# nightgoodl/ovmono3d

Hardware: AMD Instinct MI355X
Metric: images/sec/GPU @512x512 DINOv2-L SFP; AP3D delta vs reference (higher is better)
Workload: dtype f16x3; 1 GPU; DINOv2 vitl14 + SFP + ROIHeads3DGDINO (native GroundingDINO Swin-B/BERT-base, 900 queries, 6 categories -> NMS) + ROIAlign + CubeHead + decode, batch 1/GPU, 512x512 synthetic -> network res 532 -> canvas 896 (T=4097), random-init weights (seed 0); precision=f16x3, parallelism=dp1 (image-sharded, no data-path collective)

## Files before the change

include/ovm3d.h:

```cpp
#ifndef OVM3D_H
#define OVM3D_H

#include <stddef.h>
#include <stdint.h>

#ifdef __cplusplus
extern "C" {
#endif

#define OVM_OK 0
#define OVM_ERR_INVALID (-1)
#define OVM_ERR_HIP (-2)
#define OVM_ERR_MISSING_WEIGHT (-3)
#define OVM_ERR_SHAPE (-4)
#define OVM_ERR_CAPACITY (-5)
#define OVM_ERR_UNSUPPORTED (-6)

#define OVM_REC_FLOATS 48

typedef struct OvmHandle OvmHandle;
typedef void* ovm_stream_t;

typedef struct OvmConfig {
  int32_t embed_dim, depth, heads;
// ... 104 lines not shown
int ovm_op_gemm_swiglu(const uint16_t* a_hi, const uint16_t* a_lo, int32_t lda, const uint16_t* w_hi, const uint16_t* w_lo,
                       int32_t M, int32_t Hs, int32_t K, const float* bias, uint16_t* out_hi, uint16_t* out_lo, int32_t ldo,
                       int32_t precision, ovm_stream_t stream);
typedef struct OvmGemmEpiOp {
  int32_t epi, amode, precision, a_il, route, ksplit_hint;
  int32_t M, N, K, cH, cW, cC;
  const float* A; const float* W; const float* bias;
  const float* gamma; float* X; const int32_t* row_map; int32_t ldx, relu;
  float* C; int32_t ldc, ldo;
  float* O; int64_t o_elems; int32_t o_il, relu_o;
  const float* R; const float* R2; int32_t ldr, ldr2, padH, padW;
  float* Q; float* Kout; float* Vt; int32_t T, Tpad, heads; float qscale;
  const float* pos; int32_t G2, G, Cout, reserved;
} OvmGemmEpiOp;
int ovm_op_gemm_epi(const OvmGemmEpiOp* op, ovm_stream_t stream);
int ovm_op_interleave(const uint16_t* hi, const uint16_t* lo, int64_t rows, int32_t K, uint16_t* out, ovm_stream_t stream);
int ovm_op_layernorm(const float* x, int32_t M, int32_t D, const float* gamma, const float* beta, float eps,
                     float* y, ovm_stream_t stream);
int ovm_op_attention(const float* qkv, int32_t B, int32_t T, int32_t heads, float* out, int32_t precision,
                     ovm_stream_t stream);
int ovm_op_roi_align(const float* p2, const float* p3, const float* p4, const int32_t* hw ,
                     const float* scales , int32_t C, int32_t out_res, int32_t min_level, int32_t max_level,
                     const float* boxes, const int32_t* image_idx, int32_t n, float* out ,
                     ovm_stream_t stream);
int ovm_op_cube_decode(const float* head13, int32_t ld, const float* boxes, const float* scores, const int32_t* classes,
                       const int32_t* image_idx, const OvmImage* images, int32_t B, int32_t n, float virtual_focal,
                       int32_t postprocess, OvmDet3D* rec, int32_t* keep, ovm_stream_t stream);
int ovm_op_nms(const float* boxes, const float* scores, int32_t n, float thresh, int32_t* keep_idx, int32_t* n_keep,
               ovm_stream_t stream);
int ovm_op_rpn_proposals(const float* const* levels_o, int32_t nlev, const int32_t* sides, const float* strides,
// ... 337 lines not shown
```

ovmono3d_amd/csrc/gdino.hip:

```cpp
#include <cmath>
#include <cstdio>
#include <cstdlib>
#include "det2d.hpp"
#include "dec_chain.hpp"
#include "gdino_model.hpp"

using namespace ovm;
using namespace ovm::gdino;

namespace ovm {
GdinoTune g_gdino_tune = {1, 1, 0, 1, 1};
void set_gdino_branches(int v) { g_gdino_tune.branches = v ? 1 : 0; }
void set_gdino_dec_chain(int v) { g_gdino_tune.dec_chain = v ? 1 : 0; }
void set_gdino_ffn_split(int v) { g_gdino_tune.ffn_split = v ? 1 : 0; }
void set_gdino_swin_fused(int v) { g_gdino_tune.swin_fused = v ? 1 : 0; }
void set_gdino_gemm256(int v) { g_gdino_tune.gemm256 = v ? 1 : 0; }
}

namespace ovm {
namespace gdino {
namespace {

struct Feat { float* f; int h, w, C; };
struct DecScratch {
  float *tkv_all, *val_all;
  float *sine, *qh, *qpos, *qk, *vq, *ctx, *pre, *ow, *ffb, *b1, *b2, *delta;
  float* refs[2];
  bool chain; int ffn_chunks;
  float *ffn_x, *ffn_part;
};
struct State {
// ... 77 lines not shown
    a.scale = 1.0f / sqrtf((float)dh);
    if (r.go()) r.chk(launch_swin_qkv_attn(a, r.s_main), "swin_qkv_attn");
  } else {
    float* qkv = r.f32((size_t)M * 3 * C);
    { GemmParams q = r.gp(xw, M, blk.qkv); q.C = qkv; q.ldc = 3 * C; r.gemm(q, EPI_STORE); }
    AttnF32Params a; memset(&a, 0, sizeof(a));
    a.q = qkv; a.k = qkv + C; a.v = qkv + 2 * C; a.ldq = a.ldk = a.ldv = 3 * C;
    a.sq1 = a.sk1 = a.sv1 = (long)ws2 * 3 * C; a.sq2 = a.sk2 = a.sv2 = dh;
    a.ohi = ctx.hi; a.olo = ctx.lo; a.ldoh = ctx.ld; a.soh1 = (long)ws2 * ctx.ld; a.soh2 = dh;
    a.nb1 = nW; a.nb2 = nh; a.Tq = ws2; a.Tk = ws2; a.DH = dh; a.scale = 1.0f / sqrtf((float)dh);
    a.bias_h = blk.relbias; a.sbh = (long)ws2 * ws2; a.ldbh = ws2;
    a.bias_b = wmaps.mask; a.sbb = (long)ws2 * ws2; a.ldbb = ws2;
    r.attn(a);
  }
  { GemmParams q = r.gp(ctx, M, blk.proj); q.X = x; q.ldx = C; q.row_map = wmaps.win; r.gemm(q, EPI_RESID); }
  const bool wide = ((ntok + 127) / 128) * ((4 * C + 127) / 128) > 512 && (4 * C) % 256 == 0;
  SplitBuf hn = wide ? r.split_for256((size_t)ntok, C) : r.split((size_t)ntok, C);
  r.ln(x, ntok, C, blk.ln2, eps, nullptr, nullptr, &hn);
  SplitBuf f1 = r.split((size_t)ntok, 4 * C);
  { GemmParams q = r.gp(hn, ntok, blk.fc1); q.Ohi = f1.hi; q.Olo = f1.lo; q.ldo = f1.ld; r.gemm(q, EPI_GELU); }
  { GemmParams q = r.gp(f1, ntok, blk.fc2); q.X = x; q.ldx = C; r.gemm(q, EPI_RESID); }
  r.release(mk);
}

float* patch_merge(Run& r, const SwinStage& stg, const StageGeo& ge, const float* x, int C) {
  const int h2 = ge.h2, w2 = ge.w2;
  float* xn = r.f32((size_t)h2 * w2 * 2 * C);
  const size_t mk = r.mark();
  SplitBuf xm = r.split((size_t)h2 * w2, 4 * C);
  RowOpParams p = Run::rows(x, C, h2 * w2, 4 * C); Run::into(p, xm);
// ... 54 lines not shown
    RowOpParams p = Run::rows(f.f, f.C, n, K); Run::into(p, a);
    if (conv) { p.idx = pl->conv_map; p.nidx = 9; p.seg = f.C; }
    r.rowop(p);
    GemmParams q = r.gp(a, n, g->inproj[l].w); q.C = y; q.ldc = D;
    r.gemm(q, EPI_STORE);
    if (r.go()) r.chk(ovm_g_groupnorm(y, 1, n, D, 32, g->inproj[l].gn.g, g->inproj[l].gn.b, 1e-5f, st.vis0 + (size_t)pl->lstart[l] * D, r.s_main), "groupnorm");
  }
  r.release(mk);
}

struct EncBufs {
  float* v; SplitBuf vsp; float *t, *qvv, *tkv; SplitBuf cv; float* ct;
  BiAttnWs bw; float *sc, *stat, *part, *bml;
  float *text2, *tqk, *tv, *tctx, *tff;
  SplitBuf vis_sp, visp_sp; float *val, *ow; SplitBuf dsp; float* pre; SplitBuf ff;
};

void fusion_layer(Run& r, const EncLayer& ly, EncBufs& b, const float* vis_in, const float* text_in) {
  const OvmGdinoConfig& c = r.g->cfg;
  const int D = c.d_model, T = r.pl->T, S = r.pl->S, HF = c.heads / 2, E = c.ffn_dim / 2, dhf = E / HF;
  r.ln(vis_in, S, D, ly.lnv, c.eps, nullptr, b.v, &b.vsp);
  r.ln(text_in, T, D, ly.lnt, c.eps, nullptr, b.t);
  { GemmParams q = r.gp(b.vsp, S, ly.vqv); q.C = b.qvv; q.ldc = 2 * E; r.gemm(q, EPI_STORE); }
  r.lin(b.t, nullptr, D, T, ly.tkv, 0, nullptr, 0, b.tkv, 2 * E);
  if (!r.go()) return;
  BiAttnParams a; memset(&a, 0, sizeof(a));
  a.qv = b.qvv; a.ldq = 2 * E; a.kt = b.tkv; a.ldk = 2 * E; a.vv = b.qvv + E; a.ldvv = 2 * E; a.vt = b.tkv + E; a.ldvt = 2 * E;
  a.S = S; a.T = T; a.H = HF; a.dh = dhf; a.scale = 1.0f / sqrtf((float)dhf);
  a.cv_hi = b.cv.hi; a.cv_lo = b.cv.lo; a.ldcv = b.cv.ld; a.ct = b.ct; a.sc = b.sc; a.stat = b.stat; a.part = b.part; a.chunk = b.bw.chunk; a.nchunk = b.bw.nchunk;
  if (b.bml) { a.bm = b.bml; a.bl = b.bml + b.bw.ml; }
// ... 18 lines not shown

void deformable_layer(Run& r, const EncLayer& ly, EncBufs& b, float* vis) {
  const OvmGdinoConfig& c = r.g->cfg; Plan* pl = r.pl;
  const int D = c.d_model, S = pl->S, NOW = now_cols(c);
  { GemmParams q = r.gp(b.cv, S, ly.ov); q.C = vis; q.ldc = D; q.R = b.v; q.ldr = D; r.gemm(q, EPI_STORE); }
  {
    RowOpParams p = Run::rows(vis, D, S, D); Run::into(p, b.vis_sp);
    p.add = pl->pos; p.ld_add = D; p.add_rows = S; p.hi2 = b.visp_sp.hi; p.lo2 = b.visp_sp.lo; p.ldh2 = b.visp_sp.ld;
    r.rowop(p);
  }
  { GemmParams q = r.gp(b.vis_sp, S, ly.msda.value); q.C = b.val; q.ldc = D; r.gemm(q, EPI_STORE); }
  { GemmParams q = r.gp(b.visp_sp, S, ly.msda.offw); q.C = b.ow; q.ldc = NOW; r.gemm(q, EPI_STORE); }
  deform(r, b.val, D, b.ow, NOW, pl->ref, 2, 0, S, nullptr, &b.dsp);
  { GemmParams q = r.gp(b.dsp, S, ly.msda.out); q.C = b.pre; q.ldc = D; q.R = vis; q.ldr = D; r.gemm(q, EPI_STORE); }
  r.ln(b.pre, S, D, ly.de_ln1, c.eps, nullptr, b.v, &b.vsp);
  { GemmParams q = r.gp(b.vsp, S, ly.de_fc1); q.Ohi = b.ff.hi; q.Olo = b.ff.lo; q.ldo = b.ff.ld; q.relu = 1; r.gemm(q, EPI_STORE); }
  { GemmParams q = r.gp(b.ff, S, ly.de_fc2); q.C = b.pre; q.ldc = D; q.R = b.v; q.ldr = D; r.gemm(q, EPI_STORE); }
  r.ln(b.pre, S, D, ly.de_ln2, c.eps, nullptr, vis);
}

void encoder(Run& r, State& st) {
  const OvmGdinoConfig& c = r.g->cfg;
  const int D = c.d_model, T = r.pl->T, S = r.pl->S, HF = c.heads / 2, E = c.ffn_dim / 2, dhf = E / HF;
  r.join();
  const size_t mk = r.mark();
  EncBufs b;
  b.v = r.f32((size_t)S * D); b.vsp = r.split_for256((size_t)S, D);
  b.t = r.f32((size_t)T * D);
  b.qvv = r.f32((size_t)S * 2 * E);
  b.tkv = r.f32((size_t)T * 2 * E);
  b.cv = r.split((size_t)S, E);
  b.ct = r.f32((size_t)T * E);
  b.bw = biattn_workspace(S, T, HF, dhf, false);
  b.sc = b.bw.sc ? r.f32(b.bw.sc) : nullptr;
  b.stat = b.bw.stat ? r.f32(b.bw.stat) : nullptr;
  b.part = r.f32(b.bw.part);
  b.bml = b.bw.ml ? r.f32(2 * b.bw.ml) : nullptr;
  b.text2 = r.f32((size_t)T * D);
  b.tqk = r.f32((size_t)T * 2 * D); b.tv = r.f32((size_t)T * D); b.tctx = r.f32((size_t)T * D);
  b.tff = r.f32((size_t)T * c.ffn_dim);
  b.vis_sp = r.split((size_t)S, D); b.visp_sp = r.split((size_t)S, D);
  b.val = r.f32((size_t)S * D);
  b.ow = r.f32((size_t)S * now_cols(c));
  b.dsp = r.split((size_t)S, D);
  b.pre = r.f32((size_t)S * D);
  b.ff = r.split((size_t)S, c.ffn_dim);
  const float* vis_in = st.vis0; const float* text_in = st.text0;
  for (auto& ly : r.g->enc) {
    fusion_layer(r, ly, b, vis_in, text_in);
    vis_in = st.vis; text_in = st.text;
    text_enhancer(r, ly, b, st.text);
    deformable_layer(r, ly, b, st.vis);
    r.join();
  }
  r.release(mk);
  r.tap("source_flatten", st.vis0, (int64_t)S * D);
  r.tap("enc_vision", st.vis, (int64_t)S * D);
  r.tap("enc_text", st.text, (int64_t)T * D);
}

void select_queries(Run& r, State& st) {
// ... 292 lines not shown
    if (r) { delete pl; return r; }
    pl->arena_cap = dry.peak + 4096;
    void* q = nullptr;
    if (hipMalloc(&q, pl->arena_cap) != hipSuccess) { delete pl; g->err = "arena allocation failed"; return OVM_ERR_HIP; }
    pl->allocs.push_back(q); pl->arena = (char*)q; pl->bytes += pl->arena_cap;
    evict_plans(g, pl);
  }
  g->plans.push_front(pl);
  g->last = pl;
  OVM_TRY(g, ovm_g_normalize_image(image, g->cfg.pixel_mean, g->cfg.pixel_std, g->cfg.flip_channels, pl->img, s));
  if (pl->exec) {
    OVM_HIP(g, hipGraphLaunch(pl->exec, s));
  } else {
    Run run{g, pl, s, false};
    OVM_TRY(g, forward_impl(run));
    pl->launches = run.launches;
    if (g->graphs_enabled) capture_plan(g, pl, s);
  }
  g->launches_last = pl->launches;
  const size_t nl = (size_t)g->cfg.num_queries * g->cfg.max_text_len;
  if (pred_logits) OVM_HIP(g, hipMemcpyAsync(pred_logits, pl->out_logits, nl * sizeof(float), hipMemcpyDeviceToDevice, s));
  if (pred_boxes) OVM_HIP(g, hipMemcpyAsync(pred_boxes, pl->out_boxes, (size_t)g->cfg.num_queries * 4 * sizeof(float), hipMemcpyDeviceToDevice, s));
  return OVM_OK;
}

int ovm_gdino_detect(OvmGdino* g, const OvmImage* image, const int32_t* token_ids, int32_t ntok, const int32_t* spans, int32_t n_phrases,
                     float box_threshold, float nms_threshold, float* out_boxes, float* out_scores, int32_t* out_classes, int32_t* n_out,
                     ovm_stream_t stream) {
  int r = ovm_gdino_forward(g, image, token_ids, ntok, nullptr, nullptr, nullptr, stream);
  if (r) return r;
  Plan* pl = g->last;
// ... 2 lines not shown
}

int32_t ovm_gdino_num_queries(const OvmGdino* g) { return g ? g->cfg.num_queries : 0; }

int ovm_gdino_last_outputs(OvmGdino* g, const float** pred_logits, const float** pred_boxes, int32_t* logits_ld) {
  if (!g || !g->last) return OVM_ERR_INVALID;
  if (pred_logits) *pred_logits = g->last->out_logits;
  if (pred_boxes) *pred_boxes = g->last->out_boxes;
  if (logits_ld) *logits_ld = g->cfg.max_text_len;
  return OVM_OK;
}

int64_t ovm_gdino_debug_copy(OvmGdino* g, const char* name, void* dst, int64_t capacity_elems, ovm_stream_t stream) {
  if (!g || !g->last || !name) return OVM_ERR_INVALID;
  if (std::string(name) == "launches") return g->launches_last;
  if (std::string(name) == "plans") return (int64_t)g->plans.size();
  if (std::string(name) == "plan_bytes") { int64_t b = 0; for (Plan* q : g->plans) b += (int64_t)q->bytes; return b; }
  auto it = g->last->taps.find(name);
  if (it == g->last->taps.end()) { g->err = std::string("unknown debug tensor ") + name; return OVM_ERR_INVALID; }
  if (it->second.second > capacity_elems) return OVM_ERR_CAPACITY;
  if (hipMemcpyAsync(dst, it->second.first, (size_t)it->second.second * 4, hipMemcpyDeviceToDevice, (hipStream_t)stream) != hipSuccess) return OVM_ERR_HIP;
  return it->second.second;
}

}
```

ovmono3d_amd/csrc/gdino.hpp:

```cpp
#pragma once
#include "common.hpp"
#include "kernels.hpp"

namespace ovm {

struct RowOpParams {
  const float* x; int ldx;
  const int* idx; int nidx; int seg;
  const float* res; int ldr;
  const float* gamma; const float* beta; float eps;
  int zero_masked;
  const float* add; int ld_add; int add_rows;
  int M, D;
  float* y; int ldy;
  float* y2; int ldy2;
  half_t* hi; half_t* lo; int ldh;
  int il;
  half_t* hi2; half_t* lo2; int ldh2;
};
int launch_rowop(const RowOpParams& p, hipStream_t s);

struct AttnF32Params {
  const float *q, *k, *v; int ldq, ldk, ldv;
  long sq1, sq2, sk1, sk2, sv1, sv2;
// ... 8 lines not shown
int launch_attn_f32(const AttnF32Params& p, hipStream_t s);

struct SwinQkvAttnParams {
  const half_t* xhi; const half_t* xlo; int ldx;
  const half_t* wfrag; int KS;
  const float* bias;
  int C, nh, nW;
  const float* relbias;
  const float* mask;
  half_t* ohi; half_t* olo; int ldo;
  float scale;
};
bool swin_qkv_attn_supported(int C, int nh, int ws, int npass);
int launch_swin_qkv_attn(const SwinQkvAttnParams& p, hipStream_t s);

int launch_relpos_tables(const float* q, int ldq, int M, int H, int DH, int gh, int gw, const float* Rh, const float* Rw, float* rel_h,
                         float* rel_w, int ldrel, hipStream_t s);

struct BiAttnParams {
  const float* qv; int ldq;
  const float* kt; int ldk;
  const float* vv; int ldvv;
  const float* vt; int ldvt;
  int S, T, H, dh; float scale;
  half_t* cv_hi; half_t* cv_lo; int ldcv;
  float* cv;
  float* ct;
  float* sc;
  float* stat;
  float* part;
// ... 31 lines not shown
```

ovmono3d_amd/csrc/gdino_model.hpp:

```cpp
#pragma once
#include <hip/hip_runtime.h>
#include <array>
#include <cstring>
#include <list>
#include <map>
#include <string>
#include <vector>
#include "../../include/ovm3d.h"
#include "gdino.hpp"
#include "kernels.hpp"
#include "loader.hpp"
#include "tower.hpp"

namespace ovm {

struct GdinoTune {
  int branches;
  int dec_chain;
  int ffn_split;
  int swin_fused;
  int gemm256;
};
extern GdinoTune g_gdino_tune;

namespace gdino {

struct Lin : PackedLin {
  half_t* frag = nullptr;
  std::vector<half_t> img;
};
struct Ln { float* g = nullptr; float* b = nullptr; };
struct SplitBuf { half_t* hi = nullptr; half_t* lo = nullptr; int ld = 0; bool il = false; };

struct SwinBlock { Ln ln1, ln2; Lin qkv, proj, fc1, fc2; float* relbias = nullptr; };
struct SwinStage { std::vector<SwinBlock> blocks; int nh = 0, C = 0; bool has_red = false; Lin red; Ln dn; bool has_out = false; Ln on; };
struct BertLayer { Lin qkv, ao, fi, fo; Ln aln, oln; };
// ... 59 lines not shown
  std::vector<void*> allocs; size_t bytes = 0;
  int* d_ids = nullptr; int* d_pids = nullptr; float* text_bias = nullptr; float* text_pos = nullptr;
  int Hp = 0, Wp = 0; int* pe_map = nullptr;
  std::vector<StageGeo> geo;
  int nlev = 0; int lh[8] = {0}, lw[8] = {0}, lstart[8] = {0}; int S = 0;
  int* conv_map = nullptr; int conv_h = 0, conv_w = 0;
  float* pos = nullptr; float* ref = nullptr; float* prop_logit = nullptr; int* valid_idx = nullptr;
  float* img = nullptr;
  char* arena = nullptr; size_t arena_cap = 0;
  float* gemm_ws = nullptr; size_t gemm_ws_cap = 0;
  unsigned long long* topk_keys = nullptr; int topk_N = 0;
  float* out_logits = nullptr; float* out_boxes = nullptr;
  std::map<std::string, std::pair<const void*, int64_t>> taps;
  hipGraph_t graph = nullptr; hipGraphExec_t exec = nullptr;
  long launches = 0;
  void drop_graph() {
    if (exec) { (void)hipGraphExecDestroy(exec); exec = nullptr; }
    if (graph) { (void)hipGraphDestroy(graph); graph = nullptr; }
  }
  ~Plan() {
    drop_graph();
    for (void* p : allocs) (void)hipFree(p);
  }
};

int build_plan(OvmGdino* g, int H, int W, const std::vector<int>& ids, const std::vector<int>& pids, Plan** out);
Plan* find_plan(OvmGdino* g, int H, int W, const std::vector<int>& ids, const std::vector<int>& pids);
void evict_plans(OvmGdino* g, const Plan* incoming);
void capture_plan(OvmGdino* g, Plan* pl, hipStream_t s);

constexpr size_t kAuxWs = (size_t)16 << 20;

struct Run {
  OvmGdino* g; Plan* pl; hipStream_t s; bool dry;
  size_t off = 0, peak = 0;
  long launches = 0;
  int rc = OVM_OK;
  hipStream_t s_main = nullptr;
  float* ws = nullptr; size_t ws_cap = 0;
  bool two() const { return g->branches && g->aux && !dry; }
  void init_streams() { s_main = s; ws = pl->gemm_ws; ws_cap = two() ? pl->gemm_ws_cap - kAuxWs : pl->gemm_ws_cap; }
  void fork() {
    if (!two() || rc != OVM_OK) return;
    if (hipEventRecord(g->ev_fork, s_main) != hipSuccess || hipStreamWaitEvent(g->aux, g->ev_fork, 0) != hipSuccess) fail(OVM_ERR_HIP, "fork");
  }
  void on_text() { if (two()) { s = g->aux; ws = (float*)((char*)pl->gemm_ws + (pl->gemm_ws_cap - kAuxWs)); ws_cap = kAuxWs; } }
  void on_image() { if (two()) { s = s_main; ws = pl->gemm_ws; ws_cap = pl->gemm_ws_cap - kAuxWs; } }
  void join() {
    if (!two()) return;
    on_image();
    if (rc != OVM_OK) return;
// ... 15 lines not shown
    const size_t bytes = rows * b.ld * sizeof(half_t);
    b.hi = (half_t*)alloc(bytes);
    b.lo = g->precision == 3 ? (half_t*)alloc(bytes) : nullptr;
    if (b.ld != K && go()) {
      if (hipMemsetAsync(b.hi, 0, bytes, s) != hipSuccess) fail(OVM_ERR_HIP, "memset");
      if (b.lo && hipMemsetAsync(b.lo, 0, bytes, s) != hipSuccess) fail(OVM_ERR_HIP, "memset");
    }
    return b;
  }
  SplitBuf split_for256(size_t rows, int K) {
    if (g->precision != 3 || K % 32 || !pl->tune.gemm256) return split(rows, K);
    SplitBuf b; b.il = true; b.ld = 2 * K;
    b.hi = (half_t*)alloc(rows * b.ld * sizeof(half_t)); b.lo = b.hi ? b.hi + 32 : nullptr;
    return b;
  }
  size_t mark() const { return off; }
  void release(size_t m) { off = m; }
  void fail(int r, const char* what) { if (rc == OVM_OK) { rc = r; if (g->err.empty()) g->err = what; } }
  void chk(int r, const char* what) { ++launches; if (r != OVM_OK) fail(r, what); }
  void tap(const std::string& name, const void* p, int64_t n) { if (!dry) pl->taps[name] = {p, n}; }

  bool go() const { return !dry && rc == OVM_OK; }
  void copy(void* dst, const void* src, size_t bytes, hipStream_t st) {
    if (go() && hipMemcpyAsync(dst, src, bytes, hipMemcpyDeviceToDevice, st) != hipSuccess) fail(OVM_ERR_HIP, "hipMemcpyAsync");
  }
  static RowOpParams rows(const float* x, int ldx, int M, int D) {
    RowOpParams p; memset(&p, 0, sizeof(p));
    p.x = x; p.ldx = ldx; p.M = M; p.D = D;
    return p;
  }
  static void into(RowOpParams& p, const SplitBuf& b) { p.hi = b.hi; p.lo = b.lo; p.ldh = b.ld; p.il = b.il ? 1 : 0; }
  void rowop(const RowOpParams& p) { if (go()) chk(launch_rowop(p, s), "rowop"); }

  GemmParams gp(const SplitBuf& A, int M, const Lin& W) {
    GemmParams p = gp_base(SplitImg{A.hi, A.lo}, A.ld, W, M);
    p.a_il = A.il ? 1 : 0; p.ws_slot = 1; p.part_ws = ws; p.part_cap = ws_cap;
    return p;
  }
  void gemm(const GemmParams& p, int epi) {
    if (!go()) return;
    if (p.a_il && gemm256_supported(p, g->precision)) chk(launch_gemm256(p, epi, 1, s), "gemm256");
    else chk(launch_gemm(p, g->precision, epi, A_ROWMAJOR, s), "gemm");
  }

  void lin(const float* A, const float* A2, int lda, int M, const Lin& W, int act, const float* R, int ldr, float* C, int ldc) {
    if (!go() || M <= 0) return;
    if (!gemm_small_supported(A, lda, W.K) || (A2 && (((uintptr_t)A2) & 15))) { fail(OVM_ERR_SHAPE, "lin: unaligned fp32 operand"); return; }
    chk(launch_gemm_small_ex(A, A2, lda, M, W.K, W.hi, W.lo, W.N, W.Kpad, W.bias, act, R, ldr, C, ldc, g->precision, ws, ws_cap, s),
        "lin");
  }
  void ln(const float* x, int M, int D, const Ln& w, float eps, const float* res, float* y, const SplitBuf* sp = nullptr) {
    RowOpParams p = rows(x, D, M, D);
    p.res = res; p.ldr = D; p.gamma = w.g; p.beta = w.b; p.eps = eps; p.y = y; p.ldy = D;
    if (sp) into(p, *sp);
    rowop(p);
  }
  void attn(const AttnF32Params& p) { if (go()) chk(launch_attn_f32(p, s), "attn_f32"); }
};

// ... 5 lines not shown
```

ovmono3d_amd/csrc/ops.hip:

```cpp
#include <hip/hip_runtime.h>
#include <cstring>
#include <vector>
#include "../../include/ovm3d.h"
#include "kernels.hpp"
#include "det2d.hpp"
#include "tower.hpp"

using namespace ovm;

namespace {
__global__ void split_kernel(const float* __restrict__ x, int64_t n, half_t* __restrict__ hi, half_t* __restrict__ lo) {
  const int64_t i = (int64_t)blockIdx.x * blockDim.x + threadIdx.x;
  if (i >= n) return;
  half_t h, l; split_f16(x[i], h, l);
  hi[i] = h;
  if (lo) lo[i] = l;
}
__global__ void qkv_layout_kernel(const float* __restrict__ qkv, int B, int T, int Tpad, int heads,
                                  half_t* Qh, half_t* Ql, half_t* Kh, half_t* Kl, half_t* Vh, half_t* Vl) {
  const int D = heads * 64;
  const int64_t i = (int64_t)blockIdx.x * blockDim.x + threadIdx.x;
  const int64_t total = (int64_t)B * T * 3 * D;
  if (i >= total) return;
  const int n = (int)(i % (3 * D)); const int64_t m = i / (3 * D);
// ... 16 lines not shown
  y[i] = (float)hi[i] + (lo ? (float)lo[i] : 0.f);
}
struct Tmp {
  std::vector<void*> p;
  template <typename Tp> Tp* get(size_t n, bool zero = false) {
    void* q = nullptr;
    if (hipMalloc(&q, n * sizeof(Tp) + 16) != hipSuccess) return nullptr;
    if (zero) hipMemset(q, 0, n * sizeof(Tp) + 16);
    p.push_back(q);
    return (Tp*)q;
  }
  ~Tmp() { for (void* q : p) hipFree(q); }
};
}

namespace ovm { void set_use_gemm256(int v); void set_gdino_branches(int v); void msdeform_set_vec(int v); void set_gdino_dec_chain(int v); void set_gdino_gemm256(int v); void set_gdino_swin_fused(int v); void set_gdino_ffn_split(int v); void gemm256_set_n192(int v); void set_gemm256_ksplit(int v); }

extern "C" {

int ovm_op_split_f16(const float* x, int64_t n, uint16_t* hi, uint16_t* lo, ovm_stream_t stream) {
  if (n <= 0) return OVM_OK;
  hipLaunchKernelGGL(split_kernel, dim3((unsigned)((n + 255) / 256)), dim3(256), 0, (hipStream_t)stream, x, n, (half_t*)hi, (half_t*)lo);
  return hipGetLastError() == hipSuccess ? OVM_OK : OVM_ERR_HIP;
}

static int g_op_gemm256 = 0;
static unsigned long long* g_gemm256_stamps = nullptr;

int ovm_op_gemm(const uint16_t* a_hi, const uint16_t* a_lo, int32_t lda, const uint16_t* w_hi, const uint16_t* w_lo,
                int32_t M, int32_t N, int32_t K, const float* bias, int32_t relu, float* c, int32_t ldc,
                int32_t precision, ovm_stream_t stream) {
// ... 131 lines not shown
  if (d->epi == EPI_QKV) {
    const int64_t bh = (int64_t)((d->M + d->T - 1) / d->T) * d->heads, nqk = bh * d->T * 64, nv = bh * 64 * d->Tpad;
    if (nv < 1) return OVM_ERR_INVALID;
    Out* q = add_out(d->Q, nqk, split); Out* k = add_out(d->Kout, nqk, split); Out* v = add_out(d->Vt, nv, split);
    if (!q || !k || !v) return OVM_ERR_HIP;
    p.Qhi = q->hi; p.Qlo = q->lo; p.Khi = k->hi; p.Klo = k->lo; p.Vhi = v->hi; p.Vlo = v->lo;
  }
  const int rc = d->route == 1 ? launch_gemm256(p, d->epi, d->ksplit_hint, s) : launch_gemm(p, d->precision, d->epi, d->amode, s);
  if (rc == OVM_OK)
    for (int i = 0; i < n_out; ++i)
      hipLaunchKernelGGL(join_kernel, grid1d(outs[i].n), dim3(256), 0, s, outs[i].hi, outs[i].lo, outs[i].n, outs[i].f);
  if (hipStreamSynchronize(s) != hipSuccess) return OVM_ERR_HIP;
  return rc;
}

int ovm_op_interleave(const uint16_t* hi, const uint16_t* lo, int64_t rows, int32_t K, uint16_t* out, ovm_stream_t stream) {
  if (rows <= 0) return OVM_OK;
  if (!hi || !lo || !out || K % 32 != 0) return OVM_ERR_INVALID;
  const long n = (long)rows * K;
  hipLaunchKernelGGL(interleave_kernel, dim3((unsigned)((n + 255) / 256)), dim3(256), 0, (hipStream_t)stream, (const half_t*)hi, (const half_t*)lo,
                     (long)rows, K, (half_t*)out);
  return hipGetLastError() == hipSuccess ? OVM_OK : OVM_ERR_HIP;
}

int ovm_op_layernorm(const float* x, int32_t M, int32_t D, const float* gamma, const float* beta, float eps, float* y,
                     ovm_stream_t stream) {
  LnOut o; memset(&o, 0, sizeof(o)); o.f32 = y; o.ldf = D;
  return launch_ln_rows(x, D, M, D, gamma, beta, eps, o, (hipStream_t)stream);
}

// ... 137 lines not shown
}

int ovm_tune_set(const char* key, int32_t value) {
  if (!key) return OVM_ERR_INVALID;
  if (!strcmp(key, "gemm_bm")) { gemm_set_force_bm(value); return OVM_OK; }
  if (!strcmp(key, "gemm_stages")) { gemm_set_stages(value); return OVM_OK; }
  if (!strcmp(key, "gemm_splitk")) { gemm_set_splitk(value); return OVM_OK; }
  if (!strcmp(key, "gemm_tail")) { gemm_set_tail_rows(value); return OVM_OK; }
  if (!strcmp(key, "attn_waves")) { attn_set_waves(value); return OVM_OK; }
  if (!strcmp(key, "attn_pp")) {
#ifndef OVM_DIAG
    if (value < 0 || value > 1) return OVM_ERR_INVALID;
#endif
    attn_set_pp(value); return OVM_OK;
  }
  if (!strcmp(key, "gdino_ffn_split")) { ovm::set_gdino_ffn_split(value); return OVM_OK; }
  if (!strcmp(key, "gdino_swin_fused")) { ovm::set_gdino_swin_fused(value); return OVM_OK; }
  if (!strcmp(key, "gdino_gemm256")) { ovm::set_gdino_gemm256(value); return OVM_OK; }
  if (!strcmp(key, "gdino_dec_chain")) { ovm::set_gdino_dec_chain(value); return OVM_OK; }
  if (!strcmp(key, "msdeform_vec")) { msdeform_set_vec(value); return OVM_OK; }
  if (!strcmp(key, "attn_q64")) { attn_set_q64(value); return OVM_OK; }
  if (!strcmp(key, "attn_prio")) { attn_set_prio(value); return OVM_OK; }
  if (!strcmp(key, "attn_lds_pad")) { attn_set_lds_pad(value); return OVM_OK; }
  if (!strcmp(key, "attn_tail")) { attn_set_tail_rows(value); return OVM_OK; }
  if (!strcmp(key, "attn_tail_split")) { attn_set_tail_split(value); return OVM_OK; }
  if (!strcmp(key, "glin_small_max_tiles")) { glinear_set_small_max_tiles(value); return OVM_OK; }
  if (!strcmp(key, "glin_target_blocks")) { gemm_small_set(value, -1); return OVM_OK; }
  if (!strcmp(key, "gbmm_tiled")) { gbmm_set_tiled(value); return OVM_OK; }
  if (!strcmp(key, "glin_stages")) { gemm_small_set_stages(value); return OVM_OK; }
  if (!strcmp(key, "glin_wpe")) { gemm_small_set_wpe(value); return OVM_OK; }
// ... 91 lines not shown
```

ovmono3d_amd/lib.py:

```python
from __future__ import annotations

import ctypes as C
import os
from typing import Dict, Iterable, List, Optional, Sequence

import numpy as np

_HERE = os.path.dirname(os.path.abspath(__file__))
LIB_PATH = os.path.join(_HERE, "libovm3d.so")

OVM_REC_FLOATS = 48


class OvmConfig(C.Structure):
    _fields_ = [
        ("embed_dim", C.c_int32), ("depth", C.c_int32), ("heads", C.c_int32),
        ("pos_grid", C.c_int32), ("canvas", C.c_int32), ("fpn_channels", C.c_int32),
        ("use_depth_fusion", C.c_int32),
        ("pixel_mean", C.c_float * 3), ("pixel_std", C.c_float * 3),
        ("num_classes", C.c_int32), ("fc_dim", C.c_int32), ("pooler_res", C.c_int32),
        ("pooler_min_level", C.c_int32), ("pooler_max_level", C.c_int32),
        ("virtual_focal", C.c_float),
        ("anchor_sizes", C.c_float * 4), ("anchor_ratios", C.c_float * 3),
        ("rpn_pre_topk", C.c_int32), ("rpn_post_topk", C.c_int32), ("rpn_nms_thresh", C.c_float),
# ... 174 lines not shown
class OvmRowOp(C.Structure):
    _fields_ = [
        ("x", C.c_void_p), ("idx", C.c_void_p), ("res", C.c_void_p), ("gamma", C.c_void_p), ("beta", C.c_void_p), ("add", C.c_void_p),
        ("ldx", C.c_int32), ("nidx", C.c_int32), ("seg", C.c_int32), ("ldr", C.c_int32), ("eps", C.c_float),
        ("zero_masked", C.c_int32), ("ld_add", C.c_int32), ("add_rows", C.c_int32),
        ("M", C.c_int32), ("D", C.c_int32),
        ("y", C.c_void_p), ("y2", C.c_void_p), ("hi", C.c_void_p), ("lo", C.c_void_p), ("hi2", C.c_void_p), ("lo2", C.c_void_p),
        ("ldy", C.c_int32), ("ldy2", C.c_int32), ("ldh", C.c_int32), ("il", C.c_int32), ("ldh2", C.c_int32), ("reserved0", C.c_int32),
    ]


EXPORTS = [
    "ovm_create", "ovm_destroy", "ovm_last_error", "ovm_version", "ovm_abi_sizeof", "ovm_backbone_forward", "ovm_cube_forward",
    "ovm_rpn_box_forward", "ovm_gather_records", "ovm_gather_counts", "ovm_host_interp_pos_embed", "ovm_host_resize_pos_embed_aa", "ovm_host_sincos_pos_embed", "ovm_host_shard_range",
    "ovm_backbone_num_levels", "ovm_backbone_level",
    "ovm_op_split_f16", "ovm_op_interleave", "ovm_op_gemm", "ovm_op_gemm_epi", "ovm_op_gemm_swiglu", "ovm_host_swiglu_perm", "ovm_op_layernorm", "ovm_op_attention", "ovm_op_roi_align",
    "ovm_op_roi_align_ex", "ovm_op_compact_records", "ovm_op_ln_rows", "ovm_op_ln_gelu_split", "ovm_op_patch_gather", "ovm_op_patch_gather_f32",
    "ovm_op_cls_init", "ovm_op_tokens_cast", "ovm_op_tokens_writeback", "ovm_op_maxpool2",
    "ovm_op_cube_decode", "ovm_op_nms", "ovm_op_rpn_proposals", "ovm_op_boxhead_post", "ovm_debug_copy", "ovm_set_corun", "ovm_profile_enable", "ovm_profile_read",
    "ovm_comm_unique_id", "ovm_comm_init", "ovm_comm_destroy", "ovm_tune_set", "ovm_gdino_postprocess", "ovm_box3d_iou", "ovm_eval_iou2d", "ovm_eval_match", "ovm_eval_iou3d", "ovm_eval_nhd", "ovm_host_pil_bilinear_coeffs", "ovm_resize_bilinear_u8", "ovm_resize_bilinear_f32",
    "ovm_g_pack_weight", "ovm_host_pack_weight", "ovm_g_linear", "ovm_g_layernorm", "ovm_g_bmm", "ovm_g_bmm2", "ovm_g_softmax", "ovm_g_softmax2", "ovm_g_eltwise", "ovm_g_gather_rows",
    "ovm_g_groupnorm", "ovm_g_biattn", "ovm_g_msdeform", "ovm_g_sine_embed", "ovm_g_normalize_image", "ovm_g_topk", "ovm_g_rowmax",
    "ovm_g_attn_f32", "ovm_g_msdeform_fused", "ovm_g_rowop",
    "ovm_gdino_create", "ovm_gdino_destroy", "ovm_gdino_last_error", "ovm_gdino_forward", "ovm_gdino_detect", "ovm_gdino_set_force_topk",
    "ovm_gdino_debug_copy", "ovm_debug_set_ptr", "ovm_gdino_num_queries", "ovm_gdino_last_outputs", "ovm_infer",
    "ovm_host_jpeg_info", "ovm_host_jpeg_entropy_decode", "ovm_jpeg_reconstruct",
    "ovm_host_scene_layout", "ovm_render_scene_workspace", "ovm_render_scene",
    "ovm_geo_default_params", "ovm_geo_last_error", "ovm_geo_lift_workspace", "ovm_geo_lift", "ovm_geo_dbscan_workspace", "ovm_geo_dbscan",
    "ovm_host_geo_box",
    "ovm_sam_create", "ovm_sam_destroy", "ovm_sam_last_error", "ovm_sam_set_image", "ovm_sam_predict_boxes_workspace", "ovm_sam_predict_boxes",
    "ovm_sam_debug_copy",
# ... 39 lines not shown
    lib.ovm_backbone_forward.argtypes = [vp, C.POINTER(OvmImage), i32, vp, i32, i32, vp, vp, vp, vp]
    lib.ovm_cube_forward.argtypes = [vp, C.POINTER(OvmImage), i32, vp, vp, vp, vp, i32, i32, vp, vp, vp]
    lib.ovm_rpn_box_forward.argtypes = [vp, C.POINTER(OvmImage), i32, vp, vp, vp, vp, vp, vp, vp]
    lib.ovm_gather_records.argtypes = [vp, i32, i32, vp, i32, vp, C.POINTER(i32), vp]
    lib.ovm_gather_counts.argtypes = [vp, i32, i32, i32, C.POINTER(i32), vp]
    lib.ovm_host_interp_pos_embed.argtypes = [vp, i32, i32, i32, vp]
    lib.ovm_host_resize_pos_embed_aa.argtypes = [vp, i32, i32, i32, vp]
    lib.ovm_host_sincos_pos_embed.argtypes = [i32, i32, vp]
    lib.ovm_backbone_num_levels.argtypes = [vp]
    lib.ovm_backbone_level.argtypes = [vp, i32, C.POINTER(vp), C.POINTER(i32), C.POINTER(f32)]
    lib.ovm_host_shard_range.argtypes = [i64, i32, i32, C.POINTER(i64), C.POINTER(i64)]
    lib.ovm_op_split_f16.argtypes = [vp, i64, vp, vp, vp]
    lib.ovm_op_interleave.argtypes = [vp, vp, i64, i32, vp, vp]
    lib.ovm_op_gemm.argtypes = [vp, vp, i32, vp, vp, i32, i32, i32, vp, i32, vp, i32, i32, vp]
    lib.ovm_op_gemm_epi.argtypes = [C.POINTER(OvmGemmEpiOp), vp]
    lib.ovm_op_gemm_swiglu.argtypes = [vp, vp, i32, vp, vp, i32, i32, i32, vp, vp, vp, i32, i32, vp]
    lib.ovm_host_swiglu_perm.argtypes = [i32, vp]
    lib.ovm_op_layernorm.argtypes = [vp, i32, i32, vp, vp, f32, vp, vp]
    lib.ovm_op_attention.argtypes = [vp, i32, i32, i32, vp, i32, vp]
    lib.ovm_op_roi_align.argtypes = [vp, vp, vp, C.POINTER(i32), C.POINTER(f32), i32, i32, i32, i32, vp, vp, i32, vp, vp]
    lib.ovm_op_cube_decode.argtypes = [vp, i32, vp, vp, vp, vp, C.POINTER(OvmImage), i32, i32, f32, i32, vp, vp, vp]
    lib.ovm_op_roi_align_ex.argtypes = [C.POINTER(vp), i32, C.POINTER(i32), C.POINTER(f32), i32, i32, i32, i32, vp, vp, i32, vp, vp, i32, vp]
    lib.ovm_op_compact_records.argtypes = [vp, vp, i32, i32, vp, vp, vp]
    lib.ovm_op_ln_rows.argtypes = [vp, i32, i32, i32, vp, vp, f32, vp, i32, vp, vp, i32, i32, i32, i32, vp]
    lib.ovm_op_ln_gelu_split.argtypes = [vp, vp, i32, i32, vp, vp, f32, vp]
    lib.ovm_op_patch_gather.argtypes = [C.POINTER(OvmImage), i32, i32, i32, i32, C.POINTER(f32), C.POINTER(f32), vp, vp, vp]
    lib.ovm_op_patch_gather_f32.argtypes = [C.POINTER(i64), i32, i32, i32, vp, vp, vp]
    lib.ovm_op_cls_init.argtypes = [vp, vp, vp, vp, i32, i32, i32, i32, vp]
    lib.ovm_op_tokens_cast.argtypes = [vp, i32, i32, i32, i32, i32, vp, vp, vp, vp]
    lib.ovm_op_tokens_writeback.argtypes = [vp, vp, i32, i32, i32, i32, vp]
# ... 140 lines not shown
```

Baseline: 51.56 images/sec.

## Fuse GroundingDINO FFN fc1+activation+fc2 into one split-hidden MFMA kernel

Adds a fused MLP kernel that computes fc1, bias and GELU/ReLU, and the fc2 partial product per 256-wide hidden chunk. The hidden activation stays in LDS, and chunk partials are reduced by the existing split-K epilogue. It is used for small Swin block MLPs and for the encoder deformable FFN when the shape limits (at most 96 output tiles) and the workspace allow, removing the round trip of the wide hidden tensor through global memory and one GEMM launch. In exchange it writes fp32 partials of size chunks×M×C, reloads the input tile once per hidden chunk, and relies on a hand-written double-buffered pipeline.

```diff
diff --git a/include/ovm3d.h b/include/ovm3d.h
--- a/include/ovm3d.h
+++ b/include/ovm3d.h
@@ -142,6 +142,9 @@
   const float* pos; int32_t G2, G, Cout, reserved;
 } OvmGemmEpiOp;
 int ovm_op_gemm_epi(const OvmGemmEpiOp* op, ovm_stream_t stream);
+int ovm_op_mlp_fused(const uint16_t* x_il, int32_t ldx, const uint16_t* w1_il, const float* b1, const uint16_t* w2_il, const float* b2,
+                     int32_t M, int32_t C, int32_t hidden, int32_t act, float* ws, int64_t ws_bytes, float* X, const float* R, float* Y,
+                     ovm_stream_t stream);
 int ovm_op_interleave(const uint16_t* hi, const uint16_t* lo, int64_t rows, int32_t K, uint16_t* out, ovm_stream_t stream);
 int ovm_op_layernorm(const float* x, int32_t M, int32_t D, const float* gamma, const float* beta, float eps,
                      float* y, ovm_stream_t stream);
diff --git a/ovmono3d_amd/csrc/gdino.hip b/ovmono3d_amd/csrc/gdino.hip
--- a/ovmono3d_amd/csrc/gdino.hip
+++ b/ovmono3d_amd/csrc/gdino.hip
@@ -9,12 +9,13 @@
 using namespace ovm::gdino;
 
 namespace ovm {
-GdinoTune g_gdino_tune = {1, 1, 0, 1, 1};
+GdinoTune g_gdino_tune = {1, 1, 0, 1, 1, 1};
 void set_gdino_branches(int v) { g_gdino_tune.branches = v ? 1 : 0; }
 void set_gdino_dec_chain(int v) { g_gdino_tune.dec_chain = v ? 1 : 0; }
 void set_gdino_ffn_split(int v) { g_gdino_tune.ffn_split = v ? 1 : 0; }
 void set_gdino_swin_fused(int v) { g_gdino_tune.swin_fused = v ? 1 : 0; }
 void set_gdino_gemm256(int v) { g_gdino_tune.gemm256 = v ? 1 : 0; }
+void set_gdino_mlp_fused(int v) { g_gdino_tune.mlp_fused = v < 0 ? 0 : (v > 2 ? 2 : v); }
 }
 
 namespace ovm {
@@ -122,6 +123,14 @@
     r.attn(a);
   }
   { GemmParams q = r.gp(ctx, M, blk.proj); q.X = x; q.ldx = C; q.row_map = wmaps.win; r.gemm(q, EPI_RESID); }
+  if (r.mlp_fused_ok(1, ntok, blk.fc1, blk.fc2, 2)) {
+    SplitBuf hn = r.split_il((size_t)ntok, C);
+    r.ln(x, ntok, C, blk.ln2, eps, nullptr, nullptr, &hn);
+    GemmParams q = r.gp(hn, ntok, blk.fc2); q.X = x; q.ldx = C;
+    r.mlp_fused(hn, ntok, blk.fc1, blk.fc2, 2, q, EPI_RESID);
+    r.release(mk);
+    return;
+  }
   const bool wide = ((ntok + 127) / 128) * ((4 * C + 127) / 128) > 512 && (4 * C) % 256 == 0;
   SplitBuf hn = wide ? r.split_for256((size_t)ntok, C) : r.split((size_t)ntok, C);
   r.ln(x, ntok, C, blk.ln2, eps, nullptr, nullptr, &hn);
@@ -206,6 +215,7 @@
   BiAttnWs bw; float *sc, *stat, *part, *bml;
   float *text2, *tqk, *tv, *tctx, *tff;
   SplitBuf vis_sp, visp_sp; float *val, *ow; SplitBuf dsp; float* pre; SplitBuf ff;
+  bool ffn_fused;
 };
 
 void fusion_layer(Run& r, const EncLayer& ly, EncBufs& b, const float* vis_in, const float* text_in) {
@@ -254,8 +264,13 @@
   deform(r, b.val, D, b.ow, NOW, pl->ref, 2, 0, S, nullptr, &b.dsp);
   { GemmParams q = r.gp(b.dsp, S, ly.msda.out); q.C = b.pre; q.ldc = D; q.R = vis; q.ldr = D; r.gemm(q, EPI_STORE); }
   r.ln(b.pre, S, D, ly.de_ln1, c.eps, nullptr, b.v, &b.vsp);
-  { GemmParams q = r.gp(b.vsp, S, ly.de_fc1); q.Ohi = b.ff.hi; q.Olo = b.ff.lo; q.ldo = b.ff.ld; q.relu = 1; r.gemm(q, EPI_STORE); }
-  { GemmParams q = r.gp(b.ff, S, ly.de_fc2); q.C = b.pre; q.ldc = D; q.R = b.v; q.ldr = D; r.gemm(q, EPI_STORE); }
+  if (b.ffn_fused) {
+    GemmParams q = r.gp(b.vsp, S, ly.de_fc2); q.C = b.pre; q.ldc = D; q.R = b.v; q.ldr = D;
+    r.mlp_fused(b.vsp, S, ly.de_fc1, ly.de_fc2, 1, q, EPI_STORE);
+  } else {
+    { GemmParams q = r.gp(b.vsp, S, ly.de_fc1); q.Ohi = b.ff.hi; q.Olo = b.ff.lo; q.ldo = b.ff.ld; q.relu = 1; r.gemm(q, EPI_STORE); }
+    { GemmParams q = r.gp(b.ff, S, ly.de_fc2); q.C = b.pre; q.ldc = D; q.R = b.v; q.ldr = D; r.gemm(q, EPI_STORE); }
+  }
   r.ln(b.pre, S, D, ly.de_ln2, c.eps, nullptr, vis);
 }
 
@@ -284,7 +299,9 @@
   b.ow = r.f32((size_t)S * now_cols(c));
   b.dsp = r.split((size_t)S, D);
   b.pre = r.f32((size_t)S * D);
-  b.ff = r.split((size_t)S, c.ffn_dim);
+  b.ffn_fused = b.vsp.il;
+  for (auto& ly : r.g->enc) b.ffn_fused = b.ffn_fused && r.mlp_fused_ok(2, S, ly.de_fc1, ly.de_fc2, 1);
+  if (!b.ffn_fused) b.ff = r.split((size_t)S, c.ffn_dim);
   const float* vis_in = st.vis0; const float* text_in = st.text0;
   for (auto& ly : r.g->enc) {
     fusion_layer(r, ly, b, vis_in, text_in);
@@ -607,7 +624,7 @@
   } else {
     Run run{g, pl, s, false};
     OVM_TRY(g, forward_impl(run));
-    pl->launches = run.launches;
+    pl->launches = run.launches; pl->mlp_fused_sites = run.mlp_sites;
     if (g->graphs_enabled) capture_plan(g, pl, s);
   }
   g->launches_last = pl->launches;
@@ -640,6 +657,7 @@
 int64_t ovm_gdino_debug_copy(OvmGdino* g, const char* name, void* dst, int64_t capacity_elems, ovm_stream_t stream) {
   if (!g || !g->last || !name) return OVM_ERR_INVALID;
   if (std::string(name) == "launches") return g->launches_last;
+  if (std::string(name) == "mlp_fused_sites") return g->last->mlp_fused_sites;
   if (std::string(name) == "plans") return (int64_t)g->plans.size();
   if (std::string(name) == "plan_bytes") { int64_t b = 0; for (Plan* q : g->plans) b += (int64_t)q->bytes; return b; }
   auto it = g->last->taps.find(name);
diff --git a/ovmono3d_amd/csrc/gdino.hpp b/ovmono3d_amd/csrc/gdino.hpp
--- a/ovmono3d_amd/csrc/gdino.hpp
+++ b/ovmono3d_amd/csrc/gdino.hpp
@@ -46,6 +46,18 @@
 bool swin_qkv_attn_supported(int C, int nh, int ws, int npass);
 int launch_swin_qkv_attn(const SwinQkvAttnParams& p, hipStream_t s);
 
+struct MlpFusedParams {
+  const half_t* X; int ldx;
+  const half_t* W1; const float* b1;
+  const half_t* W2;
+  int M, C, hidden;
+  int act;
+  float* part; size_t part_cap;
+};
+bool mlp_fused_supported(int M, int C, int hidden, int act, int npass);
+size_t mlp_fused_ws_bytes(int M, int C, int hidden);
+int launch_mlp_fused(const MlpFusedParams& p, const GemmParams& out, int epi, hipStream_t s);
+
 int launch_relpos_tables(const float* q, int ldq, int M, int H, int DH, int gh, int gw, const float* Rh, const float* Rw, float* rel_h,
                          float* rel_w, int ldrel, hipStream_t s);
 
diff --git a/ovmono3d_amd/csrc/gdino_model.hpp b/ovmono3d_amd/csrc/gdino_model.hpp
--- a/ovmono3d_amd/csrc/gdino_model.hpp
+++ b/ovmono3d_amd/csrc/gdino_model.hpp
@@ -20,6 +20,7 @@
   int ffn_split;
   int swin_fused;
   int gemm256;
+  int mlp_fused;
 };
 extern GdinoTune g_gdino_tune;
 
@@ -109,6 +110,7 @@
   std::map<std::string, std::pair<const void*, int64_t>> taps;
   hipGraph_t graph = nullptr; hipGraphExec_t exec = nullptr;
   long launches = 0;
+  int mlp_fused_sites = 0;
   void drop_graph() {
     if (exec) { (void)hipGraphExecDestroy(exec); exec = nullptr; }
     if (graph) { (void)hipGraphDestroy(graph); graph = nullptr; }
@@ -130,6 +132,7 @@
   OvmGdino* g; Plan* pl; hipStream_t s; bool dry;
   size_t off = 0, peak = 0;
   long launches = 0;
+  int mlp_sites = 0;
   int rc = OVM_OK;
   hipStream_t s_main = nullptr;
   float* ws = nullptr; size_t ws_cap = 0;
@@ -175,6 +178,11 @@
     b.hi = (half_t*)alloc(rows * b.ld * sizeof(half_t)); b.lo = b.hi ? b.hi + 32 : nullptr;
     return b;
   }
+  SplitBuf split_il(size_t rows, int K) {
+    SplitBuf b; b.il = true; b.ld = 2 * K;
+    b.hi = (half_t*)alloc(rows * b.ld * sizeof(half_t)); b.lo = b.hi + 32;
+    return b;
+  }
   size_t mark() const { return off; }
   void release(size_t m) { off = m; }
   void fail(int r, const char* what) { if (rc == OVM_OK) { rc = r; if (g->err.empty()) g->err = what; } }
@@ -204,6 +212,23 @@
     else chk(launch_gemm(p, g->precision, epi, A_ROWMAJOR, s), "gemm");
   }
 
+  bool mlp_fused_ok(int site, int M, const Lin& fc1, const Lin& fc2, int act) const {
+    const int C = fc2.N, hidden = fc1.N;
+    if (pl->tune.mlp_fused < site || g->precision != 3 || fc1.K != C || fc1.Kpad != C || fc2.K != hidden || fc2.Kpad != hidden) return false;
+    if (!mlp_fused_supported(M, C, hidden, act, g->precision)) return false;
+    if ((long)((M + 127) / 128) * ((C + 127) / 128) > 96) return false;
+    const size_t cap = (g->branches && g->aux) ? pl->gemm_ws_cap - kAuxWs : pl->gemm_ws_cap;
+    return mlp_fused_ws_bytes(M, C, hidden) <= cap;
+  }
+  void mlp_fused(const SplitBuf& A, int M, const Lin& fc1, const Lin& fc2, int act, const GemmParams& out, int epi) {
+    ++mlp_sites;
+    if (!go()) return;
+    MlpFusedParams p; memset(&p, 0, sizeof(p));
+    p.X = A.hi; p.ldx = A.ld; p.W1 = fc1.hi; p.b1 = fc1.bias; p.W2 = fc2.hi; p.M = M; p.C = fc2.N; p.hidden = fc1.N; p.act = act;
+    p.part = ws; p.part_cap = ws_cap;
+    chk(launch_mlp_fused(p, out, epi, s), "mlp_fused");
+  }
+
   void lin(const float* A, const float* A2, int lda, int M, const Lin& W, int act, const float* R, int ldr, float* C, int ldc) {
     if (!go() || M <= 0) return;
     if (!gemm_small_supported(A, lda, W.K) || (A2 && (((uintptr_t)A2) & 15))) { fail(OVM_ERR_SHAPE, "lin: unaligned fp32 operand"); return; }
diff --git a/ovmono3d_amd/csrc/mlp_fused.hip b/ovmono3d_amd/csrc/mlp_fused.hip
--- /dev/null
+++ b/ovmono3d_amd/csrc/mlp_fused.hip
@@ -0,0 +1,189 @@
+#include <hip/hip_runtime.h>
+#include "gemm.hpp"
+#include "gdino.hpp"
+
+namespace ovm {
+
+namespace {
+
+constexpr int kBM = 64;
+constexpr int kHC = 256;
+constexpr int kKG = kHC / 32;
+constexpr int kBN = 256;
+constexpr int kSlot = (kBM + 256) * 128;
+constexpr int kOffW = kBM * 128;
+constexpr int kOffH = 2 * kSlot;
+constexpr int kHGroup = kBM * 128;
+constexpr int kSmem = kOffH + kKG * kHGroup;
+static_assert(kSmem <= 160 * 1024 && kSlot % 16 == 0 && kOffH % 16 == 0, "LDS map");
+
+__device__ __forceinline__ int frag_off(int row, int chunk) { return row * 128 + (chunk ^ ((row >> 1) & 7)) * 16; }
+
+template <int ACT>
+__global__ __launch_bounds__(512) void mlp_fused_kernel(const MlpFusedParams p) {
+  extern __shared__ __attribute__((aligned(16))) char smem[];
+  const int tid = threadIdx.x, lane = tid & 63;
+  const int wave = __builtin_amdgcn_readfirstlane(tid >> 6);
+  const int chunks = p.hidden / kHC;
+  const int chunk = (int)blockIdx.x % chunks, m0 = ((int)blockIdx.x / chunks) * kBM;
+  const int N = p.C;
+  const int S1 = p.C / 32;
+  const int S = S1 + ((N + kBN - 1) / kBN) * kKG;
+  const size_t ldw1 = 2 * (size_t)p.C, ldw2 = 2 * (size_t)p.hidden;
+
+  const int srow = lane >> 3, sslot = lane & 7;
+  size_t aoff, w1off[4];
+  int w2row[4], w2col[4];
+  {
+    const int row = wave * 8 + srow;
+    int m = m0 + row; if (m > p.M - 1) m = p.M - 1;
+    aoff = (size_t)m * p.ldx + (sslot ^ ((row >> 1) & 7)) * 8;
+  }
+#pragma unroll
+  for (int q = 0; q < 4; ++q) {
+    const int row = (wave + 8 * q) * 8 + srow;
+    const int ch = sslot ^ ((row >> 1) & 7);
+    w1off[q] = (size_t)(chunk * kHC + row) * ldw1 + ch * 8;
+    w2row[q] = row;
+    w2col[q] = chunk * kKG * 64 + ch * 8;
+  }
+  auto stage = [&](int s) {
+    char* base = smem + (s & 1) * kSlot;
+    if (s < S1) {
+      glds16(p.X + aoff + (size_t)s * 64, base + wave * 1024);
+#pragma unroll
+      for (int q = 0; q < 4; ++q) glds16(p.W1 + w1off[q] + (size_t)s * 64, base + kOffW + (wave + 8 * q) * 1024);
+    } else {
+      const int s2 = s - S1, nb = s2 / kKG, g = s2 % kKG;
+#pragma unroll
+      for (int q = 0; q < 4; ++q) {
+        int n = nb * kBN + w2row[q]; if (n > N - 1) n = N - 1;
+        glds16(p.W2 + (size_t)n * ldw2 + w2col[q] + g * 64, base + kOffW + (wave + 8 * q) * 1024);
+      }
+    }
+  };
+
+  const int fr = lane & 15, fq = lane >> 4;
+  const int wm = wave >> 2, wn = wave & 3;
+  int oa_hi[2], oa_lo[2], ow_hi[4], ow_lo[4];
+#pragma unroll
+  for (int mi = 0; mi < 2; ++mi) {
+    const int row = wm * 32 + mi * 16 + fr;
+    oa_hi[mi] = frag_off(row, fq); oa_lo[mi] = frag_off(row, 4 + fq);
+  }
+#pragma unroll
+  for (int ni = 0; ni < 4; ++ni) {
+    const int row = wn * 64 + ni * 16 + fr;
+    ow_hi[ni] = kOffW + frag_off(row, fq); ow_lo[ni] = kOffW + frag_off(row, 4 + fq);
+  }
+  f32x4 acc[2][4];
+  auto zero = [&]() {
+#pragma unroll
+    for (int mi = 0; mi < 2; ++mi)
+#pragma unroll
+      for (int ni = 0; ni < 4; ++ni) acc[mi][ni] = (f32x4){0.f, 0.f, 0.f, 0.f};
+  };
+  auto mma = [&](const char* abase, const char* wbase) {
+    half8 ah[2], al[2], wh[4], wl[4];
+#pragma unroll
+    for (int mi = 0; mi < 2; ++mi) { ah[mi] = *(const half8*)(abase + oa_hi[mi]); al[mi] = *(const half8*)(abase + oa_lo[mi]); }
+#pragma unroll
+    for (int ni = 0; ni < 4; ++ni) { wh[ni] = *(const half8*)(wbase + ow_hi[ni]); wl[ni] = *(const half8*)(wbase + ow_lo[ni]); }
+#pragma unroll
+    for (int ni = 0; ni < 4; ++ni)
+#pragma unroll
+      for (int mi = 0; mi < 2; ++mi) {
+        f32x4 c = acc[mi][ni];
+        c = __builtin_amdgcn_mfma_f32_16x16x32_f16(wl[ni], ah[mi], c, 0, 0, 0);
+        c = __builtin_amdgcn_mfma_f32_16x16x32_f16(wh[ni], al[mi], c, 0, 0, 0);
+        c = __builtin_amdgcn_mfma_f32_16x16x32_f16(wh[ni], ah[mi], c, 0, 0, 0);
+        acc[mi][ni] = c;
+      }
+  };
+
+  zero();
+  stage(0);
+  asm volatile("s_waitcnt vmcnt(0)" ::: "memory");
+  __syncthreads();
+  for (int s = 0; s < S; ++s) {
+    if (s + 1 < S) stage(s + 1);
+    const char* slot = smem + (s & 1) * kSlot;
+    if (s < S1) {
+      mma(slot, slot);
+      if (s == S1 - 1) {
+#pragma unroll
+        for (int ni = 0; ni < 4; ++ni) {
+          const int hc = wn * 64 + ni * 16 + fq * 4;
+          const f32x4 b = p.b1 ? *(const f32x4*)(p.b1 + chunk * kHC + hc) : (f32x4){0.f, 0.f, 0.f, 0.f};
+          char* hg = smem + kOffH + (hc >> 5) * kHGroup + (fq & 1) * 8;
+          const int c = (ni & 1) * 2 + (fq >> 1);
+#pragma unroll
+          for (int mi = 0; mi < 2; ++mi) {
+            const int row = wm * 32 + mi * 16 + fr;
+            half4 h, l;
+#pragma unroll
+            for (int r = 0; r < 4; ++r) {
+              const float z = acc[mi][ni][r] + b[r];
+              half_t hh, ll; split_f16(ACT == 2 ? gelu_erf(z) : fmaxf(z, 0.f), hh, ll); h[r] = hh; l[r] = ll;
+            }
+            *(half4*)(hg + frag_off(row, c)) = h;
+            *(half4*)(hg + frag_off(row, 4 + c)) = l;
+          }
+        }
+        zero();
+      }
+    } else {
+      const int s2 = s - S1, nb = s2 / kKG, g = s2 % kKG;
+      mma(smem + kOffH + g * kHGroup, slot);
+      if (g == kKG - 1) {
+#pragma unroll
+        for (int mi = 0; mi < 2; ++mi) {
+          const int m = m0 + wm * 32 + mi * 16 + fr;
+#pragma unroll
+          for (int ni = 0; ni < 4; ++ni) {
+            const int n = nb * kBN + wn * 64 + ni * 16 + fq * 4;
+            if (m < p.M && n < N) *(f32x4*)(p.part + ((size_t)chunk * p.M + m) * N + n) = acc[mi][ni];
+          }
+        }
+        zero();
+      }
+    }
+    asm volatile("s_waitcnt vmcnt(0)" ::: "memory");
+    __syncthreads();
+  }
+}
+
+}
+
+bool mlp_fused_supported(int M, int C, int hidden, int act, int npass) {
+  return npass == 3 && M >= 1 && C >= 32 && C % 32 == 0 && hidden >= kHC && hidden % kHC == 0 && (act == 1 || act == 2) &&
+         ((long)(M + kBM - 1) / kBM) * (hidden / kHC) <= 0x7fffffffL;
+}
+
+size_t mlp_fused_ws_bytes(int M, int C, int hidden) { return (size_t)(hidden / kHC) * M * C * sizeof(float); }
+
+int launch_mlp_fused(const MlpFusedParams& p, const GemmParams& out, int epi, hipStream_t s) {
+  if (!mlp_fused_supported(p.M, p.C, p.hidden, p.act, 3) || (epi != EPI_RESID && epi != EPI_STORE)) return OVM_ERR_INVALID;
+  if (!p.X || !p.W1 || !p.W2 || !p.part || p.ldx < 2 * p.C || p.ldx % 8 != 0) return OVM_ERR_INVALID;
+  if ((((uintptr_t)p.X) | ((uintptr_t)p.W1) | ((uintptr_t)p.W2) | ((uintptr_t)p.part) | ((uintptr_t)p.b1)) & 15) return OVM_ERR_INVALID;
+  if (epi == EPI_RESID ? !out.X : (!out.C && !out.Ohi)) return OVM_ERR_INVALID;
+  if (p.part_cap < mlp_fused_ws_bytes(p.M, p.C, p.hidden)) return OVM_ERR_CAPACITY;
+  const int chunks = p.hidden / kHC, tiles = (p.M + kBM - 1) / kBM;
+  static bool attr_set = false;
+  if (!attr_set) {
+    if (hipFuncSetAttribute((const void*)mlp_fused_kernel<1>, hipFuncAttributeMaxDynamicSharedMemorySize, kSmem) != hipSuccess ||
+        hipFuncSetAttribute((const void*)mlp_fused_kernel<2>, hipFuncAttributeMaxDynamicSharedMemorySize, kSmem) != hipSuccess)
+      return OVM_ERR_HIP;
+    attr_set = true;
+  }
+  if (p.act == 2) hipLaunchKernelGGL((mlp_fused_kernel<2>), dim3(tiles * chunks), dim3(512), kSmem, s, p);
+  else hipLaunchKernelGGL((mlp_fused_kernel<1>), dim3(tiles * chunks), dim3(512), kSmem, s, p);
+  GemmParams q = out;
+  q.M = p.M; q.N = p.C; q.K = p.hidden; q.ksplit = chunks; q.kchunk = kKG; q.part = p.part;
+  const long n = (long)p.M * (p.C / 4);
+  if (epi == EPI_RESID) hipLaunchKernelGGL((splitk_epilogue_kernel<EPI_RESID>), dim3((unsigned)((n + 255) / 256)), dim3(256), 0, s, q);
+  else hipLaunchKernelGGL((splitk_epilogue_kernel<EPI_STORE>), dim3((unsigned)((n + 255) / 256)), dim3(256), 0, s, q);
+  return hipGetLastError() == hipSuccess ? OVM_OK : OVM_ERR_HIP;
+}
+
+}
diff --git a/ovmono3d_amd/csrc/ops.hip b/ovmono3d_amd/csrc/ops.hip
--- a/ovmono3d_amd/csrc/ops.hip
+++ b/ovmono3d_amd/csrc/ops.hip
@@ -4,6 +4,7 @@
 #include "../../include/ovm3d.h"
 #include "kernels.hpp"
 #include "det2d.hpp"
+#include "gdino.hpp"
 #include "tower.hpp"
 
 using namespace ovm;
@@ -54,7 +55,7 @@
 };
 }
 
-namespace ovm { void set_use_gemm256(int v); void set_gdino_branches(int v); void msdeform_set_vec(int v); void set_gdino_dec_chain(int v); void set_gdino_gemm256(int v); void set_gdino_swin_fused(int v); void set_gdino_ffn_split(int v); void gemm256_set_n192(int v); void set_gemm256_ksplit(int v); }
+namespace ovm { void set_use_gemm256(int v); void set_gdino_branches(int v); void msdeform_set_vec(int v); void set_gdino_dec_chain(int v); void set_gdino_gemm256(int v); void set_gdino_swin_fused(int v); void set_gdino_ffn_split(int v); void set_gdino_mlp_fused(int v); void gemm256_set_n192(int v); void set_gemm256_ksplit(int v); }
 
 extern "C" {
 
@@ -216,6 +217,20 @@
   return rc;
 }
 
+int ovm_op_mlp_fused(const uint16_t* x_il, int32_t ldx, const uint16_t* w1_il, const float* b1, const uint16_t* w2_il, const float* b2,
+                     int32_t M, int32_t C, int32_t hidden, int32_t act, float* ws, int64_t ws_bytes, float* X, const float* R, float* Y,
+                     ovm_stream_t stream) {
+  if (!mlp_fused_supported(M, C, hidden, act, 3) || ws_bytes < 0 || (!X && !Y)) return OVM_ERR_INVALID;
+  MlpFusedParams p; memset(&p, 0, sizeof(p));
+  p.X = (const half_t*)x_il; p.ldx = ldx; p.W1 = (const half_t*)w1_il; p.b1 = b1; p.W2 = (const half_t*)w2_il;
+  p.M = M; p.C = C; p.hidden = hidden; p.act = act; p.part = ws; p.part_cap = (size_t)ws_bytes;
+  GemmParams q; memset(&q, 0, sizeof(q));
+  q.bias = b2;
+  if (X) { q.X = X; q.ldx = C; return launch_mlp_fused(p, q, EPI_RESID, (hipStream_t)stream); }
+  q.C = Y; q.ldc = C; q.R = R; q.ldr = C;
+  return launch_mlp_fused(p, q, EPI_STORE, (hipStream_t)stream);
+}
+
 int ovm_op_interleave(const uint16_t* hi, const uint16_t* lo, int64_t rows, int32_t K, uint16_t* out, ovm_stream_t stream) {
   if (rows <= 0) return OVM_OK;
   if (!hi || !lo || !out || K % 32 != 0) return OVM_ERR_INVALID;
@@ -383,6 +398,7 @@
 #endif
     attn_set_pp(value); return OVM_OK;
   }
+  if (!strcmp(key, "gdino_mlp_fused")) { ovm::set_gdino_mlp_fused(value); return OVM_OK; }
   if (!strcmp(key, "gdino_ffn_split")) { ovm::set_gdino_ffn_split(value); return OVM_OK; }
   if (!strcmp(key, "gdino_swin_fused")) { ovm::set_gdino_swin_fused(value); return OVM_OK; }
   if (!strcmp(key, "gdino_gemm256")) { ovm::set_gdino_gemm256(value); return OVM_OK; }
diff --git a/ovmono3d_amd/lib.py b/ovmono3d_amd/lib.py
--- a/ovmono3d_amd/lib.py
+++ b/ovmono3d_amd/lib.py
@@ -212,7 +212,7 @@
     "ovm_create", "ovm_destroy", "ovm_last_error", "ovm_version", "ovm_abi_sizeof", "ovm_backbone_forward", "ovm_cube_forward",
     "ovm_rpn_box_forward", "ovm_gather_records", "ovm_gather_counts", "ovm_host_interp_pos_embed", "ovm_host_resize_pos_embed_aa", "ovm_host_sincos_pos_embed", "ovm_host_shard_range",
     "ovm_backbone_num_levels", "ovm_backbone_level",
-    "ovm_op_split_f16", "ovm_op_interleave", "ovm_op_gemm", "ovm_op_gemm_epi", "ovm_op_gemm_swiglu", "ovm_host_swiglu_perm", "ovm_op_layernorm", "ovm_op_attention", "ovm_op_roi_align",
+    "ovm_op_split_f16", "ovm_op_interleave", "ovm_op_gemm", "ovm_op_gemm_epi", "ovm_op_mlp_fused", "ovm_op_gemm_swiglu", "ovm_host_swiglu_perm", "ovm_op_layernorm", "ovm_op_attention", "ovm_op_roi_align",
     "ovm_op_roi_align_ex", "ovm_op_compact_records", "ovm_op_ln_rows", "ovm_op_ln_gelu_split", "ovm_op_patch_gather", "ovm_op_patch_gather_f32",
     "ovm_op_cls_init", "ovm_op_tokens_cast", "ovm_op_tokens_writeback", "ovm_op_maxpool2",
     "ovm_op_cube_decode", "ovm_op_nms", "ovm_op_rpn_proposals", "ovm_op_boxhead_post", "ovm_debug_copy", "ovm_set_corun", "ovm_profile_enable", "ovm_profile_read",
@@ -282,6 +282,7 @@
     lib.ovm_op_interleave.argtypes = [vp, vp, i64, i32, vp, vp]
     lib.ovm_op_gemm.argtypes = [vp, vp, i32, vp, vp, i32, i32, i32, vp, i32, vp, i32, i32, vp]
     lib.ovm_op_gemm_epi.argtypes = [C.POINTER(OvmGemmEpiOp), vp]
+    lib.ovm_op_mlp_fused.argtypes = [vp, i32, vp, vp, vp, vp, i32, i32, i32, i32, vp, i64, vp, vp, vp, vp]
     lib.ovm_op_gemm_swiglu.argtypes = [vp, vp, i32, vp, vp, i32, i32, i32, vp, vp, vp, i32, i32, vp]
     lib.ovm_host_swiglu_perm.argtypes = [i32, vp]
     lib.ovm_op_layernorm.argtypes = [vp, i32, i32, vp, vp, f32, vp, vp]
```

Result: faster. 55.01 images/sec (median of 6 runs) (+6.7%).
